# src-d/kmcuda

Measured on AMD Instinct MI355X. Metric: point-assignments/sec per Lloyd iter (8Mx256@1024), higher is better.
Workload: dtype f32

## Files before the change

kmcuda_amd/csrc/engine.cpp:

```cpp
#include "engine.hpp"

#include <math.h>
#include <stdio.h>
#include <stdlib.h>
#include <string.h>

#include <mutex>
#include <vector>

#include "../../include/kmcuda_amd.h"

namespace kmx {

int g_verbosity = 0;

namespace {
std::mutex g_stream_pool_mutex;
std::vector<std::vector<hipStream_t>> g_stream_pool;
}

hipStream_t pooled_stream_acquire(int device) {
  {
    std::lock_guard<std::mutex> lock(g_stream_pool_mutex);
    if ((size_t)device < g_stream_pool.size() && !g_stream_pool[device].empty()) {
// ... 43 lines not shown
  if (!pinned_) {
    if (hipHostMalloc(reinterpret_cast<void **>(&pinned_), kPinnedWords * sizeof(uint32_t), hipHostMallocCoherent) != hipSuccess) {
      pinned_ = nullptr;
      return nullptr;
    }
    memset(pinned_, 0, kPinnedWords * sizeof(uint32_t));
    void *dp = nullptr;
    if (hipHostGetDevicePointer(&dp, pinned_, 0) != hipSuccess || dp == nullptr) {
      (void)hipHostFree(pinned_);
      pinned_ = nullptr;
      pinned_dev_ = nullptr;
      return nullptr;
    }
    pinned_dev_ = static_cast<uint32_t *>(dp);
  }
  n = (n + 3u) & ~(size_t)3u;
  if (pinned_used_ + n > kPinnedWords) return nullptr;
  uint32_t *r = pinned_ + pinned_used_;
  if (dev_addr) *dev_addr = pinned_dev_ + pinned_used_;
  pinned_used_ += n;
  return r;
}

Engine::~Engine() {
  if (device_ >= 0) (void)hipSetDevice(device_);
  for (auto &s : spans_) { (void)hipEventDestroy(s.a); (void)hipEventDestroy(s.b); }
  for (void *p : owned_) (void)hipFree(p);
  if (pinned_) (void)hipHostFree(pinned_);
  if (side_stream_ && own_side_stream_) pooled_stream_release(device_, side_stream_);
  if (ev_fork_) (void)hipEventDestroy(ev_fork_);
  if (ev_join_) (void)hipEventDestroy(ev_join_);
  for (hipEvent_t e : ev_report_)
    if (e) (void)hipEventDestroy(e);
  if (ev_rows_) (void)hipEventDestroy(ev_rows_);
  if (own_stream_ && stream_) {
    if (blocking_stream_) (void)hipStreamDestroy(stream_);
    else pooled_stream_release(device_, stream_);
  }
}

int Engine::init(int device, uint32_t n_rows, uint32_t D, uint32_t K, int metric, int fp16x2, hipStream_t stream) {
  if (getenv("KMCUDA_AMD_DEBUG")) g_verbosity = atoi(getenv("KMCUDA_AMD_DEBUG"));
  if (const char *f = getenv("KMCUDA_AMD_FILTER")) filter_mode_ = strcmp(f, "f32") == 0 ? 1 : 0;
  if (const char *c = getenv("KMCUDA_AMD_ROW_CACHE")) row_cache_allowed_ = atoi(c) != 0;
  carry_pairs_ = true;
  if (const char *c = getenv("KMCUDA_AMD_CARRY_PAIRS")) carry_pairs_ = atoi(c) != 0;
  if (const char *c = getenv("KMCUDA_AMD_SETTLE")) settle_ = atoi(c) != 0;
  if (const char *c = getenv("KMCUDA_AMD_DUO")) { duo_on_ = atoi(c) != 0; duo_always_ = atoi(c) == 2; }
  if (const char *c = getenv("KMCUDA_AMD_COARSE_MFMA")) coarse_mfma_ = atoi(c) == 32 ? 32u : 16u;
  if (const char *c = getenv("KMCUDA_AMD_WIDE")) wide_ok_ = atoi(c) != 0;
  if (const char *c = getenv("KMCUDA_AMD_GEMM")) wide_ok_ = atoi(c) != 0;
  if (const char *u = getenv("KMCUDA_AMD_UPDATE"))
    ms_.force = strcmp(u, "radix") == 0 ? 1 : (strcmp(u, "sync") == 0 ? 2 : (strcmp(u, "bucket") == 0 ? 3 : 0));
  if (D == 0 || K < 1 || K >= 0x7FFFFFFFu) return kInvalidArguments;
  if (fp16x2) return kInvalidArguments;
  int ndev = 0;
  if (hipGetDeviceCount(&ndev) != hipSuccess || device < 0 || device >= ndev) return kNoSuchDevice;
  KMX_HIP(hipSetDevice(device), kNoSuchDevice);
  device_ = device;
  if (stream == (hipStream_t)(intptr_t)-1) {
    KMX_HIP(hipStreamCreateWithFlags(&stream_, hipStreamDefault), kRuntimeError);
    own_stream_ = true;
    blocking_stream_ = true;
  } else if (stream) {
    stream_ = stream;
  } else {
    stream_ = pooled_stream_acquire(device);
    if (!stream_) return kRuntimeError;
    own_stream_ = true;
  }
  N_ = n_rows; D_ = D; K_ = K; metric_ = metric; fp16x2_ = fp16x2;
  K_pad_ = (K + 31) / 32 * 32;
  Kt_ = (K + 63) / 64 * 64;
  DP_ = lloyd_dp_for(D);
  long wide_min_d = 257;
  if (const char *c = getenv("KMCUDA_AMD_WIDE_MIN_D")) {
    const long d = atol(c);
    if (d > 0) wide_min_d = d;
  }
  if (wide_ok_ && (long)D >= wide_min_d) DP_ = 0;
  eps_ = (float)(1.02 * ((double)D + 12.0) * ldexp(1.0, -24));
  tie_slack_ = metric == 0 ? 0.f : 1e-6f;

  wide_dp_ = (DP_ == 0 && wide_ok_) ? (D + 63) / 64 * 64 : 0;
  const uint32_t dp = DP_ ? DP_ : (wide_dp_ ? wide_dp_ : 8);
  int rc;
  if ((rc = alloc(&csqr_, K))) return rc;
  if ((rc = alloc(&bias_, K_pad_))) return rc;
  if ((rc = alloc(&bias2_, K_pad_))) return rc;
  if ((rc = alloc(&cfil_, (size_t)K_pad_ * dp))) return rc;
  if ((rc = alloc(&ct_, (size_t)D * Kt_))) return rc;
  if ((rc = alloc(&stats_base_, 16))) return rc;
  stats_ = stats_base_;
  if ((rc = alloc(&mu_, dp))) return rc;
  if ((rc = alloc(&finite_, Kt_))) return rc;
  if ((rc = alloc(&flagged_, n_rows))) return rc;
  if ((rc = alloc(&pairs_, 3 * (size_t)n_rows))) return rc;
  if ((rc = alloc(&counters_, 16))) return rc;
  if ((rc = alloc(&keys_tmp_, 2 * (size_t)n_rows))) return rc;
  if ((rc = alloc(&vals_tmp_, 2 * (size_t)n_rows))) return rc;
  if ((rc = alloc(&keys_sorted_, 2 * (size_t)n_rows))) return rc;
  if ((rc = alloc(&rows_sorted_, 2 * (size_t)n_rows))) return rc;
  if ((rc = alloc(&offsets2_, 2 * (size_t)K + 2))) return rc;
  if ((rc = alloc(&move_blocks_, (size_t)n_rows / 1024 + 4))) return rc;
  if ((rc = alloc(&bucket_work_, move_bucket_words(K)))) return rc;
  KMX_HIP(hipMemsetAsync(bucket_work_, 0, move_bucket_words(K) * sizeof(uint32_t), stream_), kRuntimeError);
// ... 1005 lines not shown
```

kmcuda_amd/csrc/kernels.hpp:

```cpp
#pragma once
#include <hip/hip_runtime.h>
#include <stdint.h>
#include "launch_dispatch.hpp"

namespace kmx {

struct LloydArgs {
  const float *samples;
  uint32_t N, D, K;
  uint32_t K_pad;
  uint32_t DP;
  uint32_t Kt;
  const float *cfil;
  const float *bias;
  const float *mu;
  const float *ct;
  const float *csqr;
  const uint32_t *stats;
  float eps;
  float tie_slack;
  uint32_t *assignments, *assignments_prev;
  uint32_t *flagged;
  uint32_t *pairs;
  uint32_t *counters;
// ... 45 lines not shown
                                       float *cfil, void *panelhi, uint32_t *stats, uint32_t *stats_next,
                                       uint32_t *zero_a, uint32_t *zero_b, uint32_t *zero_c,
                                       float *drift ,
                                       uint32_t *zero_d , hipStream_t st);
hipError_t launch_apply_prep_frozen(const double *delta, const double *dcount_d, float *centroids, uint32_t *ccounts,
                                    const StopCtl &stop, uint32_t K, uint32_t D, uint32_t K_pad, uint32_t DP,
                                    const float *mu, uint32_t *finite, float *bias, float *bias2, float *cfil,
                                    void *panelhi, uint32_t *stats, uint32_t *stats_next, uint32_t *zero_a,
                                    uint32_t *zero_b, uint32_t *zero_c, float *drift, uint32_t *zero_d, hipStream_t st);
hipError_t launch_lloyd_coarse_carry(const LloydArgs &a, const void *rows, bool half_rows, const void *xcache,
                                     const float *xmeta, const void *panelhi, uint32_t *undecided, float *und_thr,
                                     const CarryArgs &cy, uint32_t rows_hint, uint32_t *duo, hipStream_t st);
hipError_t launch_carry_skip(uint32_t N, uint32_t K, const uint32_t *assignments, uint32_t *assignments_prev,
                             const CarryArgs &cy, const float *xmeta, const float *drift, const uint32_t *stats,
                             float tie_slack, uint32_t *row_list, const uint32_t *finite, uint32_t *pairs,
                             uint32_t *counters, bool probe, hipStream_t st, uint32_t wide_dg = 0);
hipError_t launch_centroid_rows(int metric, const float *centroids, uint32_t K, uint32_t D, uint32_t Kt, float *csqr,
                                float *ct, hipStream_t st);
hipError_t launch_lloyd_coarse(const LloydArgs &a, const void *rows, bool half_rows, const void *xcache,
                               const float *xmeta, const void *panelhi, uint32_t *undecided, float *und_thr,
                               uint32_t *duo, hipStream_t st);
hipError_t launch_lloyd_duo(const LloydArgs &a, const uint32_t *duo, hipStream_t st, const CarryArgs *cy = nullptr);
hipError_t launch_lloyd_refine(const LloydArgs &a, const void *rows, bool half_rows, const void *panelhi,
                               const uint32_t *row_list, const float *thr_list, const uint32_t *n_list,
                               uint32_t rows_hint , hipStream_t st);
hipError_t launch_lloyd_refine_carry(const LloydArgs &a, const void *rows, bool half_rows, const void *panelhi,
                                     const uint32_t *row_list, const float *thr_list, const uint32_t *n_list,
                                     uint32_t rows_hint, const CarryArgs &cy, hipStream_t st);
hipError_t launch_row_cache(const void *rows, bool half_rows, uint32_t N, uint32_t D, uint32_t DP, const float *mu,
                            void *xcache, float *xmeta, hipStream_t st);

hipError_t launch_row_halves(const void *rows, bool half_rows, uint32_t N, uint32_t D, uint32_t DG, const float *mu,
                             void *xg, float *meta , hipStream_t st);
size_t wide_cont_words(uint32_t N);
hipError_t launch_lloyd_wide(const LloydArgs &a, const void *xg, const float *meta, uint32_t DG ,
                             const void *panelhi, uint32_t *undecided, float *und_thr, uint32_t *und_cont, hipStream_t st,
                             const CarryArgs *cy = nullptr);
hipError_t launch_wide_contenders(int metric, const LloydArgs &a, const float *centroids, uint32_t DG,
                                  const uint32_t *und_rows, const uint32_t *und_cont, hipStream_t st);

size_t sort_temp_bytes(size_t n, uint32_t max_key);
uint32_t move_bucket_stride(uint32_t K);
size_t move_bucket_words(uint32_t K);
uint32_t move_bucket_cap(uint32_t N, uint32_t K);
hipError_t launch_inverse_assignments(const uint32_t *assignments, uint32_t N, uint32_t K, uint32_t *keys_tmp,
                                      uint32_t *vals_tmp, uint32_t *keys_sorted, uint32_t *inv,
                                      uint32_t *offsets, void *temp, size_t temp_bytes, hipStream_t st);
struct MoveState {
  uint32_t *host = nullptr;
  uint32_t *host_dev = nullptr;
  uint32_t last_events = 0xFFFFFFFFu;
  int force = 0;
  uint32_t n_radix = 0, n_direct = 0;
};
struct MoveWeights {
  const float *weights;
  double *dweight;
  double *win;
};
hipError_t launch_move_deltas(const float *samples, uint32_t N, uint32_t D, uint32_t K, const uint32_t *prev,
                              const uint32_t *cur, uint32_t *keys_tmp, uint32_t *vals_tmp, uint32_t *keys_sorted,
                              uint32_t *rows_sorted, uint32_t *offsets2, void *temp, size_t temp_bytes,
                              uint32_t *bucket_rows, uint32_t cap, double *delta, int32_t *dcount ,
                              double *tail ,
                              const uint32_t *counters, uint32_t *blockoff, uint32_t *bucket_work, MoveState *ms,
                              hipStream_t st, const MoveWeights *mw = nullptr);
hipError_t launch_adjust_exact(int metric, const float *samples, uint32_t N, uint32_t D, uint32_t K,
                               const uint32_t *prev, const uint32_t *cur, uint32_t *keys_tmp, uint32_t *vals_tmp,
                               uint32_t *keys_sorted, uint32_t *rows_sorted, uint32_t *offsets2, void *temp,
                               size_t temp_bytes, float *work, float *centroids, uint32_t *ccounts, hipStream_t st);
hipError_t launch_apply_delta(int metric, const double *delta, const int32_t *dcount ,
                              const double *dcount_d , uint32_t K, uint32_t D,
                              float *centroids, uint32_t *ccounts, const StopCtl &stop, hipStream_t st,
                              const double *wtail = nullptr ,
                              double *cweights = nullptr );
size_t weights_check_doubles();
hipError_t launch_weights_check(const float *weights, uint32_t N, double *work, hipStream_t st);
hipError_t launch_sum_buffers(double *const *bufs_dev, uint32_t nbuf, size_t len, hipStream_t st);

hipError_t preload_update_code();
hipError_t preload_lloyd_f16_code();
hipError_t preload_lloyd_code();
hipError_t preload_lloyd_carry_code();
hipError_t preload_lloyd_duo_code();
hipError_t launch_gather_rows(const float *samples, const uint32_t *idx, uint32_t K, uint32_t D, float *out, hipStream_t st);
hipError_t launch_kmpp_step(int metric, const float *samples, uint32_t N, uint32_t D, const float *centroid,
                            uint32_t cc, float *dists, hipStream_t st);
struct KmppOutlierBuf {
  uint32_t *ecut = nullptr;
  void *outl = nullptr;
  uint32_t *outl_count = nullptr;
};
size_t kmpp_outlier_bytes();
size_t kmpp_totals_bytes();
hipError_t launch_kmpp_step2(int metric, const float *samples, uint32_t N, uint32_t D, const float *centroid,
                             uint32_t cc, float *dists, void *block_stats, double *bpre, void *totals,
                             const uint32_t *fail, const KmppOutlierBuf &out, hipStream_t st,
                             const float *weights = nullptr, float *terms = nullptr);
hipError_t launch_kmpp_weigh(const float *dists, const float *weights, uint32_t N, float *terms, const uint32_t *fail,
                             hipStream_t st);
constexpr int kKmppMaxShards = 16;
struct KmppShardPtrs {
  const float *dists;
  const double *bpre;
  void *totals;
  const float *samples;
// ... 295 lines not shown
```

kmcuda_amd/csrc/kmcuda_api.cpp:

```cpp
#include <dlfcn.h>
#include <math.h>
#include <stdio.h>
#include <stdlib.h>
#include <string.h>

#include <algorithm>
#include <chrono>
#include <cmath>
#include <condition_variable>
#include <functional>
#include <memory>
#include <mutex>
#include <thread>
#include <vector>

#include "../../include/kmcuda.h"
#include "../../include/kmcuda_amd.h"
#include "engine.hpp"
#include "knn_host.hpp"

using namespace kmx;

#define INFO(...) do { if (verbosity > 0) { printf(__VA_ARGS__); } } while (false)
#define DEBUG(...) do { if (verbosity > 1) { printf(__VA_ARGS__); } } while (false)
// ... 1499 lines not shown
  int ndev = 0;
  (void)hipGetDeviceCount(&ndev);
  return ndev < 32 && device > (1u << ndev);
}

void sync_callers_device(int32_t device_ptrs) {
  if (device_ptrs >= 0 && hipSetDevice(device_ptrs) == hipSuccess) (void)hipDeviceSynchronize();
}

int check_kmeans_args(const KmeansSwitches &sw, KMCUDAInitMethod init, float tolerance, float yinyang_t,
                      uint32_t samples_size, uint16_t features_size, uint32_t clusters_size, uint32_t device,
                      int32_t fp16x2, int32_t verbosity, const float *samples, const float *centroids,
                      const uint32_t *assignments, const float *sample_weights) {
  if (clusters_size < 2 || clusters_size == UINT32_MAX) return kmcudaInvalidArguments;
  if (features_size == 0) return kmcudaInvalidArguments;
  if (samples_size < clusters_size) return kmcudaInvalidArguments;
  if (device_mask_refused(device)) return kmcudaNoSuchDevice;
  if (samples == nullptr || centroids == nullptr || assignments == nullptr) return kmcudaInvalidArguments;
  if (tolerance < 0 || tolerance > 1) return kmcudaInvalidArguments;
  if (yinyang_t < 0 || yinyang_t > 0.5) return kmcudaInvalidArguments;
  if (!sample_weights) return kmcudaSuccess;
  if (init == kmcudaInitMethodAFKMC2 || sw.exact_update || (fp16x2 && sw.fp16_strict)) {
    INFO("sample weights are not supported with afkmc2, KMCUDA_AMD_EXACT_UPDATE=1 or KMCUDA_AMD_FP16_STRICT=1\n");
    return kmcudaInvalidArguments;
  }
  if (init == kmcudaInitMethodParallel) {
    INFO("sample weights are not supported with k-means||\n");
    return kmcudaInvalidArguments;
  }
  return kmcudaSuccess;
}

int seed_parallel_first(KMCUDAInitMethod *init, const void *init_params, KMCUDADistanceMetric metric,
                        uint32_t samples_size, uint16_t features_size, uint32_t clusters_size, uint32_t seed,
                        int first_device, int32_t device_ptrs, int32_t fp16x2, int32_t verbosity, const float *samples,
                        float *centroids) {
  if (*init != kmcudaInitMethodParallel) return kmcudaSuccess;
  const auto *sp = static_cast<const kmamd_seed_parallel_params *>(init_params);
  INFO("performing k-means||...\n");
  RETERR(kmamd_kmeans_seed_parallel(metric, samples_size, fp16x2 ? (uint16_t)(2u * features_size) : features_size,
                                    clusters_size, sp ? sp->rounds : 0u, sp ? sp->oversampling : 0.f, seed,
                                    device_ptrs >= 0 ? device_ptrs : first_device, device_ptrs, fp16x2, verbosity, samples,
                                    centroids, nullptr, nullptr, 0, nullptr, nullptr, nullptr));
  kmx::g_verbosity = verbosity;
  *init = kmcudaInitMethodImport;
  return kmcudaSuccess;
}

void publish_run_stats(Job &job, std::chrono::steady_clock::time_point t_loop) {
  job.stats.loop_seconds = std::chrono::duration<double>(std::chrono::steady_clock::now() - t_loop).count();
  job.collective_collect();
  if (job.sw.update_trace)
    for (auto &s : job.shards)
      fprintf(stderr, "[update] shard on device %d: %u radix, %u direct; loop %.4f s\n", s->dev, s->eng->ms_.n_radix, s->eng->ms_.n_direct,
              job.stats.loop_seconds);
  std::lock_guard<std::mutex> lock(g_last_run_mutex);
  g_last_run = job.stats;
}

}

extern "C" {

KMCUDAResult kmeans_cuda(KMCUDAInitMethod init, const void *init_params, float tolerance, float yinyang_t,
                         KMCUDADistanceMetric metric, uint32_t samples_size, uint16_t features_size,
                         uint32_t clusters_size, uint32_t seed, uint32_t device, int32_t device_ptrs, int32_t fp16x2,
                         int32_t verbosity, const float *samples, float *centroids, uint32_t *assignments,
                         float *average_distance) {
  return static_cast<KMCUDAResult>(kmamd_kmeans_weighted(init, init_params, tolerance, yinyang_t, metric, samples_size,
                                                         features_size, clusters_size, seed, device, device_ptrs, fp16x2,
                                                         verbosity, samples, centroids, assignments, average_distance,
                                                         nullptr));
}

int kmamd_kmeans_weighted(int init_, const void *init_params, float tolerance, float yinyang_t, int metric_,
                          uint32_t samples_size, uint16_t features_size, uint32_t clusters_size, uint32_t seed,
                          uint32_t device, int32_t device_ptrs, int32_t fp16x2, int32_t verbosity, const float *samples,
                          float *centroids, uint32_t *assignments, float *average_distance,
                          const float *sample_weights) {
  KMCUDAInitMethod init = static_cast<KMCUDAInitMethod>(init_);
  const KMCUDADistanceMetric metric = static_cast<KMCUDADistanceMetric>(metric_);
  kmx::g_verbosity = verbosity;
  DEBUG("arguments: %d %p %.3f %.2f %d %u %u %u %u %u %d %d %p %p %p %p\n", init, init_params, tolerance, yinyang_t,
        metric, samples_size, (unsigned)features_size, clusters_size, seed, device, fp16x2, verbosity,
        (const void *)samples, (void *)centroids, (void *)assignments, (void *)average_distance);
  const KmeansSwitches sw = kmeans_switches();
  RETERR(check_kmeans_args(sw, init, tolerance, yinyang_t, samples_size, features_size, clusters_size, device, fp16x2,
                           verbosity, samples, centroids, assignments, sample_weights));
  INFO("reassignments threshold: %u\n", uint32_t(tolerance * samples_size));
  const uint32_t yy_groups_size = yinyang_t * clusters_size;
  DEBUG("yinyang groups: %u\n", yy_groups_size);
  auto devs = setup_devices(device, verbosity);
  if (devs.empty()) return kmcudaNoSuchDevice;
  RETERR(seed_parallel_first(&init, init_params, metric, samples_size, features_size, clusters_size, seed, devs[0],
                             device_ptrs, fp16x2, verbosity, samples, centroids));
  sync_callers_device(device_ptrs);
  PreloadThreads preload;
  for (int d : devs) preload_code_objects(d, &preload, sw);
  PhaseClock clock(sw.timing);
  const auto t_begin = clock.t_lap;
  Job job;
  clock.wait = [&job] { (void)job.sync_all(); };
  job.fp16 = fp16x2 != 0;
  job.strict_h2 = job.fp16 && sw.fp16_strict;
  const uint32_t feats = fp16x2 ? 2u * features_size : features_size;
  RETERR(job.setup(sw, devs, sw.virtual_shards, samples_size, feats, clusters_size, metric, verbosity, samples,
                   device_ptrs, nullptr, sample_weights));
  clock.lap("set-up (engines, uploads)");
// ... 68 lines not shown
```

kmcuda_amd/csrc/list_sum.hpp:

```cpp
#pragma once
#include <hip/hip_runtime.h>
#include <stdint.h>

namespace kmx {

template <bool WEIGHTED>
__device__ __forceinline__ double list_sum(const float *__restrict__ samples, const float *__restrict__ weights,
                                           uint32_t D, const uint32_t *rows, uint32_t r0, uint32_t r1, uint32_t f) {
  double a[8] = {0, 0, 0, 0, 0, 0, 0, 0};
  uint32_t r = r0;
  for (; r + 8 <= r1; r += 8) {
    float x[8], w[8];
#pragma unroll
    for (int j = 0; j < 8; j++) {
      const uint32_t row = rows[r + j];
      x[j] = samples[(size_t)row * D + f];
      if constexpr (WEIGHTED) w[j] = weights[row];
    }
#pragma unroll
    for (int j = 0; j < 8; j++) {
      if constexpr (WEIGHTED) a[j] += (double)w[j] * (double)x[j];
      else a[j] += (double)x[j];
    }
  }
  for (uint32_t j = 0; r < r1; r++, j++) {
    const uint32_t row = rows[r];
    if constexpr (WEIGHTED) a[j] += (double)weights[row] * (double)samples[(size_t)row * D + f];
    else a[j] += (double)samples[(size_t)row * D + f];
  }
  return ((a[0] + a[1]) + (a[2] + a[3])) + ((a[4] + a[5]) + (a[6] + a[7]));
}

template <bool WEIGHTED>
__device__ __forceinline__ void list_sum4(const float *__restrict__ samples, const float *__restrict__ weights,
                                          uint32_t D, const uint32_t *rows, uint32_t r0, uint32_t r1, uint32_t f,
                                          double (&out)[4]) {
  double a[4][4];
#pragma unroll
  for (int j = 0; j < 4; j++)
#pragma unroll
    for (int e = 0; e < 4; e++) a[j][e] = 0.0;
  uint32_t r = r0;
  for (; r + 4 <= r1; r += 4) {
    float4 x[4];
    double w[4] = {1.0, 1.0, 1.0, 1.0};
#pragma unroll
    for (int j = 0; j < 4; j++) {
      const uint32_t row = rows[r + j];
      x[j] = *reinterpret_cast<const float4 *>(samples + (size_t)row * D + f);
      if constexpr (WEIGHTED) w[j] = (double)weights[row];
    }
#pragma unroll
    for (int j = 0; j < 4; j++) {
      if constexpr (WEIGHTED) {
        a[j][0] += w[j] * (double)x[j].x; a[j][1] += w[j] * (double)x[j].y;
        a[j][2] += w[j] * (double)x[j].z; a[j][3] += w[j] * (double)x[j].w;
      } else {
        a[j][0] += (double)x[j].x; a[j][1] += (double)x[j].y; a[j][2] += (double)x[j].z; a[j][3] += (double)x[j].w;
      }
    }
  }
  for (uint32_t j = 0; r < r1; r++, j++) {
    const uint32_t row = rows[r];
    float4 x = *reinterpret_cast<const float4 *>(samples + (size_t)row * D + f);
    double x0 = (double)x.x, x1 = (double)x.y, x2 = (double)x.z, x3 = (double)x.w;
    if constexpr (WEIGHTED) {
      const double w = (double)weights[row];
      x0 *= w; x1 *= w; x2 *= w; x3 *= w;
    }
    if (j == 0) { a[0][0] += x0; a[0][1] += x1; a[0][2] += x2; a[0][3] += x3; }
    else if (j == 1) { a[1][0] += x0; a[1][1] += x1; a[1][2] += x2; a[1][3] += x3; }
    else { a[2][0] += x0; a[2][1] += x1; a[2][2] += x2; a[2][3] += x3; }
  }
#pragma unroll
  for (int e = 0; e < 4; e++) out[e] = (a[0][e] + a[1][e]) + (a[2][e] + a[3][e]);
}

}
```

kmcuda_amd/csrc/update.hip:

```cpp
#include <stdio.h>
#include <stdlib.h>
#include <string.h>

#include <algorithm>

#include <rocprim/device/device_radix_sort.hpp>

#include "exact.hpp"
#include "kernels.hpp"
#include "list_sum.hpp"

namespace kmx {

static unsigned bits_for(uint64_t maxval) {
  unsigned b = 1;
  while (b < 32 && (1ull << b) <= maxval) b++;
  return b;
}

size_t sort_temp_bytes(size_t n, uint32_t max_key) {
  size_t bytes = 0;
  (void)rocprim::radix_sort_pairs(nullptr, bytes, (const uint32_t *)nullptr, (uint32_t *)nullptr,
                                  (const uint32_t *)nullptr, (uint32_t *)nullptr, n, 0u, bits_for(max_key),
                                  (hipStream_t)0);
// ... 222 lines not shown
    bool ein, eout;
    move_flags(prev, cur, s, N, K, p, a, ein, eout);
    const unsigned long long min = __ballot(ein), mout = __ballot(eout);
    const unsigned long long lower = (1ull << lane) - 1ull;
    const uint32_t rank = (uint32_t)__popcll(min & lower) + (uint32_t)__popcll(mout & lower);
    if (lane == 0) wcnt[wave] = (uint32_t)__popcll(min) + (uint32_t)__popcll(mout);
    __syncthreads();
    uint32_t wbase = 0, all = 0;
#pragma unroll
    for (uint32_t k = 0; k < 4; k++) {
      if (k < wave) wbase += wcnt[k];
      all += wcnt[k];
    }
    const size_t at = (size_t)off + wbase + rank;
    if (ein) { keys[at] = 2u * a; vals[at] = s; }
    if (eout) { keys[at + (ein ? 1 : 0)] = 2u * p + 1u; vals[at + (ein ? 1 : 0)] = s; }
    off += all;
    __syncthreads();
  }
}

constexpr uint32_t kSumThreads = 1024;
constexpr uint32_t kBucketCapMax = 4096;

uint32_t move_bucket_cap(uint32_t N, uint32_t K) {
  uint32_t cap = 32;
  while (cap < kBucketCapMax && (uint64_t)cap * 2 * K <= (uint64_t)N) cap <<= 1;
  return cap;
}

struct SumArgs {
  const float *samples;
  uint32_t N, D, K;
  const uint32_t *prev, *cur;
  uint32_t *cursors;
  uint32_t stride;
  const uint32_t *bucket_rows;
  uint32_t cap;
  uint32_t *overflow;
  const uint32_t *rows_sorted, *offsets2;
  double *delta;
  int32_t *dcount;
  double *tail;
  const uint32_t *counters;
  uint32_t *res;
  uint32_t *host;
};

struct SumWeightArgs {
  const float *weights;
  double *dweight;
  double *win;
};

template <bool DIRECT, bool VEC4, bool WEIGHTED>
__device__ __forceinline__ void cluster_sums_body(const SumArgs &a, const SumWeightArgs &wa) {
  extern __shared__ __attribute__((aligned(16))) unsigned char sums_lds[];
  double *part = reinterpret_cast<double *>(sums_lds);
  uint32_t (*srt)[kBucketCapMax] = reinterpret_cast<uint32_t (*)[kBucketCapMax]>(sums_lds + kSumThreads * 4 * sizeof(double));
  uint32_t *part_u = reinterpret_cast<uint32_t *>(part);
  __shared__ uint32_t wcnt[16];
  __shared__ uint32_t sh_base;
  const uint32_t c = blockIdx.x, tid = threadIdx.x, lane = tid & 63, wave = tid >> 6;
  const uint32_t D = a.D;
  const uint32_t *rows[2];
  uint32_t n[2];
  if (DIRECT) {
    n[0] = a.cursors[(size_t)(2 * c) * a.stride];
    n[1] = a.cursors[(size_t)(2 * c + 1) * a.stride];
    __syncthreads();
    if (tid < 2) a.cursors[(size_t)(2 * c + tid) * a.stride] = 0u;
#pragma unroll
    for (int sg = 0; sg < 2; sg++) {
      const uint32_t cnt = n[sg], key = 2 * c + sg;
      if (cnt <= kSumThreads && cnt <= a.cap) {
        uint32_t *v = srt[sg];
        const uint32_t mine = tid < cnt ? a.bucket_rows[(size_t)key * a.cap + tid] : 0xFFFFFFFFu;
        if (tid < cnt) part_u[tid] = mine;
        __syncthreads();
        if (tid < cnt) {
          uint32_t rank = 0;
          for (uint32_t j = 0; j < cnt; j++) rank += part_u[j] < mine ? 1u : 0u;
          v[rank] = mine;
        }
        __syncthreads();
        rows[sg] = v;
      } else if (cnt <= a.cap) {
        uint32_t m = 2;
        while (m < cnt) m <<= 1;
        uint32_t *v = srt[sg];
        for (uint32_t i = tid; i < m; i += kSumThreads) v[i] = i < cnt ? a.bucket_rows[(size_t)key * a.cap + i] : 0xFFFFFFFFu;
        __syncthreads();
        if (cnt > 1) {
          for (uint32_t k = 2; k <= m; k <<= 1) {
            for (uint32_t j = k >> 1; j > 0; j >>= 1) {
              for (uint32_t i = tid; i < m; i += kSumThreads) {
                const uint32_t l = i ^ j;
                if (l > i) {
                  const uint32_t x = v[i], y = v[l];
                  const bool up = (i & k) == 0;
                  if ((x > y) == up) { v[i] = y; v[l] = x; }
                }
              }
              __syncthreads();
            }
          }
// ... 85 lines not shown
        const uint32_t cnt = n[sg], chunk = (cnt + groups - 1) / groups;
        const uint32_t r0 = min(cnt, g * chunk), r1 = min(cnt, r0 + chunk);
        double mine[4] = {0.0, 0.0, 0.0, 0.0};
        if (fv && r1 > r0) list_sum4<WEIGHTED>(a.samples, wa.weights, D, rows[sg], r0, r1, f, mine);
#pragma unroll
        for (int e = 0; e < 4; e++) part[(size_t)tid * 4 + e] = mine[e];
        __syncthreads();
        if (g == 0) {
#pragma unroll
          for (int e = 0; e < 4; e++) {
            double t = part[(size_t)lf * 4 + e];
            for (uint32_t gg = 1; gg < groups; gg++) t += part[(size_t)(gg * fl + lf) * 4 + e];
            tot[sg][e] = t;
          }
        }
        __syncthreads();
      }
      if (g == 0 && fv) {
#pragma unroll
        for (int e = 0; e < 4; e++) a.delta[(size_t)c * D + f + e] = tot[0][e] - tot[1][e];
      }
    }
  } else {
  const uint32_t fl = D > 128 ? 256u : (D > 64 ? 128u : 64u), groups = kSumThreads / fl;
  const uint32_t g = tid / fl, lf = tid % fl;
  for (uint32_t f0 = 0; f0 < D; f0 += fl) {
    const uint32_t f = f0 + lf;
    const bool fv = f < D;
    double tot[2] = {0, 0};
#pragma unroll
    for (int sg = 0; sg < 2; sg++) {
      const uint32_t cnt = n[sg], chunk = (cnt + groups - 1) / groups;
      const uint32_t r0 = min(cnt, g * chunk), r1 = min(cnt, r0 + chunk);
      part[tid] = (fv && r1 > r0) ? list_sum<WEIGHTED>(a.samples, wa.weights, D, rows[sg], r0, r1, f) : 0.0;
      __syncthreads();
      if (g == 0) {
        double t = part[lf];
        for (uint32_t gg = 1; gg < groups; gg++) t += part[gg * fl + lf];
        tot[sg] = t;
      }
      __syncthreads();
    }
    if (g == 0 && fv) a.delta[(size_t)c * D + f] = tot[0] - tot[1];
  }
  }
  if (tid == 0) {
    const int32_t dc = (int32_t)n[0] - (int32_t)n[1];
    if (a.dcount) a.dcount[c] = dc;
    if (a.tail) a.tail[c] = (double)dc;
    if constexpr (WEIGHTED) {
      wa.dweight[c] = wsum[0] - wsum[1];
      wa.win[c] = wsum[0];
    }
    atomicAdd(&a.res[0], n[0] + n[1]);
    atomicMax(&a.res[1], max(n[0], n[1]));
    __threadfence();
    const uint32_t ticket = atomicAdd(&a.res[2], 1u);
    if (ticket == gridDim.x - 1) {
      if (a.counters[kStopFlag] == 0u) {
        volatile uint32_t *h = a.host;
        h[0] = atomicAdd(&a.res[0], 0u);
        h[1] = atomicAdd(&a.res[1], 0u);
        h[2] = a.counters[4];
        h[4] = a.counters[kDuoCount];
      }
      a.res[0] = 0u; a.res[1] = 0u; a.res[2] = 0u; a.res[3] = 0u;
    }
  }
  if (a.tail && c == 0 && tid < 4) a.tail[a.K + tid] = (double)a.counters[tid];
}

template <bool DIRECT, bool VEC4>
__global__ __launch_bounds__(kSumThreads) void cluster_sums_kernel(SumArgs a) {
  cluster_sums_body<DIRECT, VEC4, false>(a, SumWeightArgs{nullptr, nullptr, nullptr});
}
template <bool DIRECT, bool VEC4>
__global__ __launch_bounds__(kSumThreads) void cluster_sums_w_kernel(SumArgs a, SumWeightArgs wa) {
  cluster_sums_body<DIRECT, VEC4, true>(a, wa);
}

__global__ __launch_bounds__(256) void weight_changed_kernel(const double *__restrict__ win, uint32_t K,
                                                             double *__restrict__ out) {
  __shared__ double red[256];
  double t = 0.0;
  for (uint32_t c = threadIdx.x; c < K; c += 256) t += win[c];
  red[threadIdx.x] = t;
  __syncthreads();
  for (uint32_t s = 128; s > 0; s >>= 1) {
    if (threadIdx.x < s) red[threadIdx.x] += red[threadIdx.x + s];
    __syncthreads();
  }
  if (threadIdx.x == 0) out[0] = red[0];
}

constexpr uint32_t kWeightBlocks = 1024;
__global__ __launch_bounds__(256) void weights_check_kernel(const float *__restrict__ w, uint32_t N, uint32_t chunk,
                                                            double *__restrict__ part) {
  __shared__ double red[256], bad[256];
  const uint32_t lo = blockIdx.x * chunk, hi = min(N, lo + chunk);
  double t = 0.0, b = 0.0;
  for (uint32_t s = lo + threadIdx.x; s < hi; s += 256) {
    const float v = w[s];
    if (v > 0.f && v < INFINITY) t += (double)v; else b += 1.0;
  }
  red[threadIdx.x] = t; bad[threadIdx.x] = b;
  __syncthreads();
  for (uint32_t s = 128; s > 0; s >>= 1) {
    if (threadIdx.x < s) { red[threadIdx.x] += red[threadIdx.x + s]; bad[threadIdx.x] += bad[threadIdx.x + s]; }
    __syncthreads();
  }
  if (threadIdx.x == 0) { part[2 * blockIdx.x] = red[0]; part[2 * blockIdx.x + 1] = bad[0]; }
}
__global__ __launch_bounds__(256) void weights_total_kernel(const double *__restrict__ part, uint32_t nb,
                                                            double *__restrict__ out) {
  __shared__ double red[256], bad[256];
  double t = 0.0, b = 0.0;
  for (uint32_t i = threadIdx.x; i < nb; i += 256) { t += part[2 * i]; b += part[2 * i + 1]; }
  red[threadIdx.x] = t; bad[threadIdx.x] = b;
  __syncthreads();
  for (uint32_t s = 128; s > 0; s >>= 1) {
    if (threadIdx.x < s) { red[threadIdx.x] += red[threadIdx.x + s]; bad[threadIdx.x] += bad[threadIdx.x + s]; }
    __syncthreads();
  }
  if (threadIdx.x == 0) { out[0] = red[0]; out[1] = bad[0]; }
}
size_t weights_check_doubles() { return 2 * (size_t)kWeightBlocks + 2; }
hipError_t launch_weights_check(const float *weights, uint32_t N, double *work, hipStream_t st) {
  const uint32_t chunk = ((N + kWeightBlocks - 1) / kWeightBlocks + 255u) / 256u * 256u;
  const uint32_t nb = chunk ? (N + chunk - 1) / chunk : 0;
  if (nb) hipLaunchKernelGGL(weights_check_kernel, dim3(nb), dim3(256), 0, st, weights, N, chunk, work + 2);
  hipLaunchKernelGGL(weights_total_kernel, dim3(1), dim3(256), 0, st, work + 2, nb, work);
  return hipGetLastError();
}

uint32_t move_bucket_stride(uint32_t K) {
  uint32_t s = 32;
  while (s > 1 && 2ull * K * s > 262144ull) s >>= 1;
  return s;
}
size_t move_bucket_words(uint32_t K) { return 2 * (size_t)K * move_bucket_stride(K) + 4; }

__global__ __launch_bounds__(256) void move_scatter_kernel(const uint32_t *__restrict__ prev,
                                                           const uint32_t *__restrict__ cur, uint32_t N, uint32_t K,
                                                           uint32_t *__restrict__ cursors, uint32_t stride,
                                                           uint32_t *__restrict__ bucket_rows, uint32_t cap) {
  const uint32_t s = blockIdx.x * 256u + threadIdx.x;
  uint32_t p, a;
  bool ein, eout;
  move_flags(prev, cur, s, N, K, p, a, ein, eout);
  if (ein) {
    const uint32_t at = atomicAdd(&cursors[(size_t)(2u * a) * stride], 1u);
    if (at < cap) bucket_rows[(size_t)(2u * a) * cap + at] = s;
  }
  if (eout) {
    const uint32_t at = atomicAdd(&cursors[(size_t)(2u * p + 1u) * stride], 1u);
    if (at < cap) bucket_rows[(size_t)(2u * p + 1u) * cap + at] = s;
  }
}

hipError_t launch_move_deltas(const float *samples, uint32_t N, uint32_t D, uint32_t K, const uint32_t *prev,
                              const uint32_t *cur, uint32_t *keys_tmp, uint32_t *vals_tmp, uint32_t *keys_sorted,
                              uint32_t *rows_sorted, uint32_t *offsets2, void *temp, size_t temp_bytes,
                              uint32_t *bucket_rows, uint32_t cap, double *delta, int32_t *dcount, double *tail,
                              const uint32_t *counters, uint32_t *blockoff, uint32_t *bucket_work, MoveState *ms,
                              hipStream_t st, const MoveWeights *mw) {
  const uint32_t stride = move_bucket_stride(K);
  SumArgs a;
  a.samples = samples; a.N = N; a.D = D; a.K = K; a.prev = prev; a.cur = cur;
  a.cursors = bucket_work; a.stride = stride; a.bucket_rows = bucket_rows; a.cap = cap;
  a.overflow = rows_sorted; a.rows_sorted = rows_sorted; a.offsets2 = offsets2;
  a.delta = delta; a.dcount = dcount; a.tail = tail; a.counters = counters;
  a.res = bucket_work + 2 * (size_t)K * stride; a.host = ms->host_dev;
  hipError_t e = hipSuccess;
  const bool vec4 = (D & 3u) == 0 && (((uintptr_t)samples) & 15u) == 0;
  const size_t sums_lds = kSumThreads * 4 * sizeof(double) + 2 * kBucketCapMax * sizeof(uint32_t);
  auto launch_sums = [&](bool direct) {
    if (mw) {
      const SumWeightArgs wa{mw->weights, mw->dweight, mw->win};
      const void *fn = direct ? (vec4 ? (const void *)cluster_sums_w_kernel<true, true> : (const void *)cluster_sums_w_kernel<true, false>)
                              : (vec4 ? (const void *)cluster_sums_w_kernel<false, true> : (const void *)cluster_sums_w_kernel<false, false>);
      if (hipFuncSetAttribute(fn, hipFuncAttributeMaxDynamicSharedMemorySize, (int)sums_lds) != hipSuccess) return;
      if (direct) {
        if (vec4) hipLaunchKernelGGL((cluster_sums_w_kernel<true, true>), dim3(K), dim3(kSumThreads), sums_lds, st, a, wa);
        else hipLaunchKernelGGL((cluster_sums_w_kernel<true, false>), dim3(K), dim3(kSumThreads), sums_lds, st, a, wa);
      } else {
        if (vec4) hipLaunchKernelGGL((cluster_sums_w_kernel<false, true>), dim3(K), dim3(kSumThreads), sums_lds, st, a, wa);
        else hipLaunchKernelGGL((cluster_sums_w_kernel<false, false>), dim3(K), dim3(kSumThreads), sums_lds, st, a, wa);
      }
      hipLaunchKernelGGL(weight_changed_kernel, dim3(1), dim3(256), 0, st, mw->win, K, mw->dweight + K);
      return;
    }
    const void *fn = direct ? (vec4 ? (const void *)cluster_sums_kernel<true, true> : (const void *)cluster_sums_kernel<true, false>)
                            : (vec4 ? (const void *)cluster_sums_kernel<false, true> : (const void *)cluster_sums_kernel<false, false>);
    if (hipFuncSetAttribute(fn, hipFuncAttributeMaxDynamicSharedMemorySize, (int)sums_lds) != hipSuccess) return;
    if (direct) {
      if (vec4) hipLaunchKernelGGL((cluster_sums_kernel<true, true>), dim3(K), dim3(kSumThreads), sums_lds, st, a);
      else hipLaunchKernelGGL((cluster_sums_kernel<true, false>), dim3(K), dim3(kSumThreads), sums_lds, st, a);
    } else {
      if (vec4) hipLaunchKernelGGL((cluster_sums_kernel<false, true>), dim3(K), dim3(kSumThreads), sums_lds, st, a);
      else hipLaunchKernelGGL((cluster_sums_kernel<false, false>), dim3(K), dim3(kSumThreads), sums_lds, st, a);
    }
  };
  const bool force_radix = ms->force == 1, force_sync = ms->force == 2, force_direct = ms->force == 3;
  const uint32_t est_max = std::max((uint32_t)ms->host[1] , ms->last_events / K);
  const bool radix = N != 0 && !force_direct &&
                     (force_radix || ms->last_events > N / 2 || est_max > cap - cap / 4);
  if (N == 0) {
    e = hipMemsetAsync(offsets2, 0, (2 * (size_t)K + 1) * sizeof(uint32_t), st);
    if (e != hipSuccess) return e;
    launch_sums(false);
  } else if (radix) {
    ms->n_radix++;
    const uint32_t nb = (N + kMoveRows - 1) / kMoveRows;
    hipLaunchKernelGGL(move_count_kernel, dim3(nb), dim3(256), 0, st, prev, cur, N, K, blockoff);
    hipLaunchKernelGGL(move_scan_kernel, dim3(1), dim3(1024), 0, st, blockoff, nb, blockoff + nb + 1);
    hipLaunchKernelGGL(move_write_kernel, dim3(nb), dim3(256), 0, st, prev, cur, N, K, blockoff, keys_tmp, vals_tmp);
    e = hipGetLastError();
    if (e != hipSuccess) return e;
    e = hipMemcpyAsync(ms->host + 3, blockoff + nb + 1, sizeof(uint32_t), hipMemcpyDeviceToHost, st);
    if (e == hipSuccess) e = hipStreamSynchronize(st);
    if (e != hipSuccess) return e;
    const uint32_t m = ms->host[3];
    if (m) {
      e = rocprim::radix_sort_pairs(temp, temp_bytes, (const uint32_t *)keys_tmp, keys_sorted,
                                    (const uint32_t *)vals_tmp, rows_sorted, (size_t)m, 0u, bits_for(2ull * K), st);
      if (e != hipSuccess) return e;
    }
    hipLaunchKernelGGL(offsets_kernel, dim3((2 * K + 1 + 255) / 256), dim3(256), 0, st, keys_sorted, m, 2 * K, offsets2);
    ms->last_events = m;
    ms->host[0] = m;
    launch_sums(false);
  } else {
    ms->n_direct++;
    hipLaunchKernelGGL(move_scatter_kernel, dim3((N + 255) / 256), dim3(256), 0, st, prev, cur, N, K, bucket_work,
                       stride, bucket_rows, cap);
    launch_sums(true);
    e = hipGetLastError();
    if (e != hipSuccess) return e;
    if (force_sync) {
      e = hipStreamSynchronize(st);
      if (e != hipSuccess) return e;
    }
    ms->last_events = ms->host[0];
  }
  return hipGetLastError();
}

template <int METRIC, bool WEIGHTED>
__device__ __forceinline__ void apply_delta_body(const double *__restrict__ delta, const int32_t *__restrict__ dcount,
                                                 const double *__restrict__ dcount_d, uint32_t D,
                                                 float *__restrict__ centroids, uint32_t *__restrict__ ccounts,
                                                 const StopCtl &ctl, const double *__restrict__ wtail,
                                                 double *__restrict__ cweights) {
  const uint32_t c = blockIdx.x;
  if (ctl.counters) {
    bool stop = ctl.counters[kStopFlag] != 0u;
    if constexpr (WEIGHTED) {
      if (ctl.threshold >= 0.f && dcount_d) stop = stop || (float)wtail[gridDim.x] <= ctl.threshold;
    } else {
      if (ctl.threshold >= 0.f && dcount_d) stop = stop || (float)(uint32_t)dcount_d[gridDim.x] <= ctl.threshold;
    }
    if (c == 0 && threadIdx.x == 0) {
      if (stop) ctl.counters[kStopFlag] = 1u;
      else if (ctl.threshold >= 0.f) ctl.counters[0] = 0u;
      if (ctl.host_tail) {
        volatile uint32_t *ht = ctl.host_tail;
        for (uint32_t i = 0; i < 4; i++) ht[i] = dcount_d ? (uint32_t)dcount_d[gridDim.x + i] : 0u;
        ht[4] = stop ? 1u : 0u;
        __threadfence_system();
        ht[5] = ctl.seq;
      }
    }
    if (stop) return;
  }
  const double *d = delta + (size_t)c * D;
  float *cen = centroids + (size_t)c * D;
  const uint32_t cnt_old = ccounts[c];
  const uint32_t cnt_new = cnt_old + (uint32_t)(dcount_d ? (int32_t)dcount_d[c] : dcount[c]);
  double w, cn;
  if constexpr (WEIGHTED) {
    w = cnt_old ? cweights[c] : 0.0;
    cn = w + wtail[c];
  } else {
    w = (double)cnt_old;
    cn = (double)cnt_new;
  }
  if (cnt_new == 0) {
    for (uint32_t f = threadIdx.x; f < D; f += blockDim.x) cen[f] = __builtin_nanf("");
  } else if (METRIC == 0) {
// ... 167 lines not shown
```

Before: 2.199 billion.

## Add two-wave per-cluster sums kernel and vectorize move scatter

Adds a 128-thread cluster_sums_wave_kernel in which one wave sums a cluster's incoming rows and the other its outgoing rows, using readlane-broadcast row ids, multiple double accumulators and in-LDS rank or bitonic sorting of bucket rows. It is used when the estimated per-cluster move list is small, and it merges the completion counters into a single 64-bit atomic. The move scatter kernel now handles four rows per thread with uint4 loads, which cuts the launched thread count. The aim is lower sums-stage cost in late Lloyd iterations where few points move, at the price of a large new code path with sort and overflow handling.

Result: no change. 2.215 billion (median of 6 runs) (+0.7%).

```diff
diff --git a/kmcuda_amd/csrc/engine.cpp b/kmcuda_amd/csrc/engine.cpp
--- a/kmcuda_amd/csrc/engine.cpp
+++ b/kmcuda_amd/csrc/engine.cpp
@@ -119,6 +119,8 @@
   if (const char *c = getenv("KMCUDA_AMD_GEMM")) wide_ok_ = atoi(c) != 0;
   if (const char *u = getenv("KMCUDA_AMD_UPDATE"))
     ms_.force = strcmp(u, "radix") == 0 ? 1 : (strcmp(u, "sync") == 0 ? 2 : (strcmp(u, "bucket") == 0 ? 3 : 0));
+  if (const char *u = getenv("KMCUDA_AMD_SUMS"))
+    ms_.sums = strcmp(u, "block") == 0 ? 1 : (strcmp(u, "wave-always") == 0 ? 2 : 0);
   if (D == 0 || K < 1 || K >= 0x7FFFFFFFu) return kInvalidArguments;
   if (fp16x2) return kInvalidArguments;
   int ndev = 0;
diff --git a/kmcuda_amd/csrc/kernels.hpp b/kmcuda_amd/csrc/kernels.hpp
--- a/kmcuda_amd/csrc/kernels.hpp
+++ b/kmcuda_amd/csrc/kernels.hpp
@@ -121,6 +121,8 @@
   uint32_t last_events = 0xFFFFFFFFu;
   int force = 0;
   uint32_t n_radix = 0, n_direct = 0;
+  int sums = 0;
+  uint32_t n_wave = 0;
 };
 struct MoveWeights {
   const float *weights;
diff --git a/kmcuda_amd/csrc/kmcuda_api.cpp b/kmcuda_amd/csrc/kmcuda_api.cpp
--- a/kmcuda_amd/csrc/kmcuda_api.cpp
+++ b/kmcuda_amd/csrc/kmcuda_api.cpp
@@ -1575,8 +1575,8 @@
   job.collective_collect();
   if (job.sw.update_trace)
     for (auto &s : job.shards)
-      fprintf(stderr, "[update] shard on device %d: %u radix, %u direct; loop %.4f s\n", s->dev, s->eng->ms_.n_radix, s->eng->ms_.n_direct,
-              job.stats.loop_seconds);
+      fprintf(stderr, "[update] shard on device %d: %u radix, %u direct, %u summed per wave; loop %.4f s\n", s->dev,
+              s->eng->ms_.n_radix, s->eng->ms_.n_direct, s->eng->ms_.n_wave, job.stats.loop_seconds);
   std::lock_guard<std::mutex> lock(g_last_run_mutex);
   g_last_run = job.stats;
 }
diff --git a/kmcuda_amd/csrc/list_sum.hpp b/kmcuda_amd/csrc/list_sum.hpp
--- a/kmcuda_amd/csrc/list_sum.hpp
+++ b/kmcuda_amd/csrc/list_sum.hpp
@@ -76,4 +76,90 @@
   for (int e = 0; e < 4; e++) out[e] = (a[0][e] + a[1][e]) + (a[2][e] + a[3][e]);
 }
 
+template <int V>
+__device__ __forceinline__ void row_load(const float *__restrict__ p, float (&x)[V]) {
+  if constexpr (V == 4) {
+    const float4 v = *reinterpret_cast<const float4 *>(p);
+    x[0] = v.x; x[1] = v.y; x[2] = v.z; x[3] = v.w;
+  } else {
+    x[0] = *p;
+  }
 }
+
+template <int V, int A, int NB, bool LROWS>
+__device__ __forceinline__ void wave_list_sum(const float *__restrict__ samples, uint32_t D, const uint32_t *rows,
+                                              uint32_t n, uint32_t groups, uint32_t f, double (&tot)[V]) {
+  static_assert(64 % NB == 0 && (A == 4 || A == 8), "window and accumulators");
+  typedef const __attribute__((address_space(3))) uint32_t *lds_rows_t;
+#pragma unroll
+  for (int e = 0; e < V; e++) tot[e] = 0.0;
+  if (n == 0) return;
+  const uint32_t lane = threadIdx.x & 63;
+  const uint32_t chunk = (n + groups - 1) / groups;
+  double acc[A][V], t[V];
+#pragma unroll
+  for (int q = 0; q < A; q++)
+#pragma unroll
+    for (int e = 0; e < V; e++) acc[q][e] = 0.0;
+#pragma unroll
+  for (int e = 0; e < V; e++) t[e] = 0.0;
+  auto ids = [&](uint32_t at) -> uint32_t {
+    const uint32_t i = min(at + lane, n - 1);
+    if constexpr (LROWS) return ((lds_rows_t)rows)[i];
+    else return rows[i];
+  };
+  uint32_t bb = 0;
+  uint32_t idc = ids(0), idn = ids(64);
+  float x[NB][V];
+#pragma unroll
+  for (int j = 0; j < NB; j++) {
+    const uint32_t row = (uint32_t)__builtin_amdgcn_readlane((int)idc, (int)min((uint32_t)j, n - 1));
+    row_load<V>(samples + (size_t)row * D + f, x[j]);
+  }
+  uint32_t pos = 0, glen = min(chunk, n), folded = 0;
+  for (uint32_t i0 = 0; i0 < n; i0 += NB) {
+    if (i0 == bb + 64) { bb += 64; idc = idn; idn = ids(bb + 64); }
+#pragma unroll
+    for (int j = 0; j < NB; j++) {
+      const uint32_t i = i0 + j;
+      double xd[V];
+#pragma unroll
+      for (int e = 0; e < V; e++) xd[e] = (double)x[j][e];
+      {
+        const uint32_t k = min(i + NB, n - 1) - bb;
+        const uint32_t r0 = (uint32_t)__builtin_amdgcn_readlane((int)idc, (int)(k & 63u));
+        const uint32_t r1 = (uint32_t)__builtin_amdgcn_readlane((int)idn, (int)(k & 63u));
+        const uint32_t row = k < 64u ? r0 : r1;
+        row_load<V>(samples + (size_t)row * D + f, x[j]);
+      }
+      if (i < n) {
+        const uint32_t sel = pos & (uint32_t)(A - 1);
+#pragma unroll
+        for (int q = 0; q < A; q++) {
+          if (sel == (uint32_t)q) {
+#pragma unroll
+            for (int e = 0; e < V; e++) acc[q][e] += xd[e];
+          }
+        }
+        if (++pos == glen) {
+#pragma unroll
+          for (int e = 0; e < V; e++) {
+            double s;
+            if constexpr (A == 4) s = (acc[0][e] + acc[1][e]) + (acc[2][e] + acc[3][e]);
+            else s = ((acc[0][e] + acc[1][e]) + (acc[2][e] + acc[3][e])) + ((acc[4][e] + acc[5][e]) + (acc[6][e] + acc[7][e]));
+            t[e] = folded ? t[e] + s : s;
+#pragma unroll
+            for (int q = 0; q < A; q++) acc[q][e] = 0.0;
+          }
+          folded++;
+          pos = 0;
+          glen = min(chunk, n - i - 1);
+        }
+      }
+    }
+  }
+#pragma unroll
+  for (int e = 0; e < V; e++) tot[e] = folded < groups ? t[e] + 0.0 : t[e];
+}
+
+}
diff --git a/kmcuda_amd/csrc/update.hip b/kmcuda_amd/csrc/update.hip
--- a/kmcuda_amd/csrc/update.hip
+++ b/kmcuda_amd/csrc/update.hip
@@ -298,6 +298,23 @@
   double *dweight;
   double *win;
 };
+
+__device__ __forceinline__ void sums_report(const SumArgs &a, uint32_t n_in, uint32_t n_out) {
+  atomicAdd(&a.res[0], n_in + n_out);
+  atomicMax(&a.res[1], max(n_in, n_out));
+  __threadfence();
+  const uint32_t ticket = atomicAdd(&a.res[2], 1u);
+  if (ticket == gridDim.x - 1) {
+    if (a.counters[kStopFlag] == 0u) {
+      volatile uint32_t *h = a.host;
+      h[0] = atomicAdd(&a.res[0], 0u);
+      h[1] = atomicAdd(&a.res[1], 0u);
+      h[2] = a.counters[4];
+      h[4] = a.counters[kDuoCount];
+    }
+    a.res[0] = 0u; a.res[1] = 0u; a.res[2] = 0u; a.res[3] = 0u;
+  }
+}
 
 template <bool DIRECT, bool VEC4, bool WEIGHTED>
 __device__ __forceinline__ void cluster_sums_body(const SumArgs &a, const SumWeightArgs &wa) {
@@ -489,20 +506,7 @@
       wa.dweight[c] = wsum[0] - wsum[1];
       wa.win[c] = wsum[0];
     }
-    atomicAdd(&a.res[0], n[0] + n[1]);
-    atomicMax(&a.res[1], max(n[0], n[1]));
-    __threadfence();
-    const uint32_t ticket = atomicAdd(&a.res[2], 1u);
-    if (ticket == gridDim.x - 1) {
-      if (a.counters[kStopFlag] == 0u) {
-        volatile uint32_t *h = a.host;
-        h[0] = atomicAdd(&a.res[0], 0u);
-        h[1] = atomicAdd(&a.res[1], 0u);
-        h[2] = a.counters[4];
-        h[4] = a.counters[kDuoCount];
-      }
-      a.res[0] = 0u; a.res[1] = 0u; a.res[2] = 0u; a.res[3] = 0u;
-    }
+    sums_report(a, n[0], n[1]);
   }
   if (a.tail && c == 0 && tid < 4) a.tail[a.K + tid] = (double)a.counters[tid];
 }
@@ -514,6 +518,175 @@
 template <bool DIRECT, bool VEC4>
 __global__ __launch_bounds__(kSumThreads) void cluster_sums_w_kernel(SumArgs a, SumWeightArgs wa) {
   cluster_sums_body<DIRECT, VEC4, true>(a, wa);
+}
+
+constexpr uint32_t kWaveThreads = 128;
+constexpr uint32_t kWaveRank = 256;
+constexpr uint32_t kWaveListMax = 1024;
+
+template <int V, int A, int NB, bool LROWS>
+__device__ __forceinline__ void wave_sums_slabs(const SumArgs &a, uint32_t c, uint32_t wave, uint32_t lane,
+                                                const uint32_t *rows, uint32_t n, uint32_t groups, double *xch) {
+  for (uint32_t f0 = 0; f0 < a.D; f0 += 64u * V) {
+    const uint32_t f = f0 + lane * V;
+    const bool fv = f < a.D;
+    double tot[V];
+    wave_list_sum<V, A, NB, LROWS>(a.samples, a.D, rows, n, groups, fv ? f : 0u, tot);
+    if (wave == 1) {
+#pragma unroll
+      for (int e = 0; e < V; e++) xch[lane * V + e] = tot[e];
+    }
+    __syncthreads();
+    if (wave == 0 && fv) {
+#pragma unroll
+      for (int e = 0; e < V; e++) a.delta[(size_t)c * a.D + f + e] = tot[e] - xch[lane * V + e];
+    }
+    __syncthreads();
+  }
+}
+template <int V, int A, int NB>
+__device__ __forceinline__ void wave_sums_run(const SumArgs &a, uint32_t c, uint32_t wave, uint32_t lane,
+                                              const uint32_t *rows_g, const uint32_t *rows_l, uint32_t n,
+                                              uint32_t groups, double *xch) {
+  if (rows_g) wave_sums_slabs<V, A, NB, false>(a, c, wave, lane, rows_g, n, groups, xch);
+  else wave_sums_slabs<V, A, NB, true>(a, c, wave, lane, rows_l, n, groups, xch);
+}
+
+__device__ __forceinline__ void wave_report(const SumArgs &a, uint32_t n_in, uint32_t n_out) {
+  uint32_t z = atomicMax(&a.res[2], max(n_in, n_out));
+  asm volatile("v_and_b32 %0, 0, %0" : "+v"(z));
+  const unsigned long long mine = ((unsigned long long)(n_in + n_out) << 32) + 1ull + z;
+  const unsigned long long old = atomicAdd(reinterpret_cast<unsigned long long *>(a.res), mine);
+  if ((uint32_t)old == gridDim.x - 1) {
+    if (a.counters[kStopFlag] == 0u) {
+      volatile uint32_t *h = a.host;
+      h[0] = (uint32_t)(old >> 32) + n_in + n_out;
+      h[1] = atomicAdd(&a.res[2], 0u);
+      h[2] = a.counters[4];
+      h[4] = a.counters[kDuoCount];
+    }
+    a.res[0] = 0u; a.res[1] = 0u; a.res[2] = 0u; a.res[3] = 0u;
+  }
+}
+
+template <bool DIRECT, bool VEC4>
+__global__ __launch_bounds__(kWaveThreads) void cluster_sums_wave_kernel(SumArgs a) {
+  __shared__ __attribute__((aligned(16))) uint32_t srt[2][kBucketCapMax];
+  __shared__ double xch[64 * 4];
+  const uint32_t c = blockIdx.x, tid = threadIdx.x, lane = tid & 63;
+  const uint32_t wave = (uint32_t)__builtin_amdgcn_readfirstlane((int)(tid >> 6));
+  uint32_t n[2];
+  const uint32_t *rows_g = nullptr;
+  if (DIRECT) {
+    n[0] = (uint32_t)__builtin_amdgcn_readfirstlane((int)a.cursors[(size_t)(2 * c) * a.stride]);
+    n[1] = (uint32_t)__builtin_amdgcn_readfirstlane((int)a.cursors[(size_t)(2 * c + 1) * a.stride]);
+    __syncthreads();
+    if (tid < 2) a.cursors[(size_t)(2 * c + tid) * a.stride] = 0u;
+    const uint32_t cnt = n[wave], key = 2 * c + wave;
+    uint32_t *v = srt[wave];
+    const int mode = cnt > a.cap ? 2 : (cnt > kWaveRank ? 1 : 0);
+    uint32_t m = 0;
+    if (mode == 0) m = (cnt + 3u) & ~3u;
+    if (mode == 1) { m = 2; while (m < cnt) m <<= 1; }
+    for (uint32_t i = lane; i < m; i += 64) v[i] = i < cnt ? a.bucket_rows[(size_t)key * a.cap + i] : 0xFFFFFFFFu;
+    __syncthreads();
+    uint32_t mine[4], rank[4] = {0, 0, 0, 0};
+    if (mode == 0) {
+#pragma unroll
+      for (int k = 0; k < 4; k++) mine[k] = lane + 64u * k < cnt ? v[lane + 64u * k] : 0u;
+      for (uint32_t j = 0; j < m; j += 4) {
+        const uint4 o = *reinterpret_cast<const uint4 *>(v + j);
+#pragma unroll
+        for (int k = 0; k < 4; k++)
+          rank[k] += (o.x < mine[k] ? 1u : 0u) + (o.y < mine[k] ? 1u : 0u) + (o.z < mine[k] ? 1u : 0u) + (o.w < mine[k] ? 1u : 0u);
+      }
+    }
+    __syncthreads();
+    if (mode == 0) {
+#pragma unroll
+      for (int k = 0; k < 4; k++)
+        if (lane + 64u * k < cnt) v[rank[k]] = mine[k];
+    }
+    const uint32_t n0 = n[0] > kWaveRank && n[0] <= a.cap ? n[0] : 0u, n1 = n[1] > kWaveRank && n[1] <= a.cap ? n[1] : 0u;
+    const uint32_t longest = max(n0, n1);
+    if (longest) {
+      uint32_t mm = 2;
+      while (mm < longest) mm <<= 1;
+      for (uint32_t k = 2; k <= mm; k <<= 1) {
+        for (uint32_t j = k >> 1; j > 0; j >>= 1) {
+          if (mode == 1 && k <= m) {
+            for (uint32_t i = lane; i < m; i += 64) {
+              const uint32_t l = i ^ j;
+              if (l > i) {
+                const uint32_t x = v[i], y = v[l];
+                const bool up = (i & k) == 0;
+                if ((x > y) == up) { v[i] = y; v[l] = x; }
+              }
+            }
+          }
+          __syncthreads();
+        }
+      }
+    }
+    if (mode == 2) {
+      uint32_t base_w = 0;
+      if (lane == 0) base_w = atomicAdd(&a.res[3], cnt);
+      base_w = (uint32_t)__builtin_amdgcn_readfirstlane((int)base_w);
+      uint32_t *dst = a.overflow + base_w;
+      uint32_t done = 0;
+      for (uint64_t base = 0; base < a.N; base += 256) {
+        uint32_t hit[4], cntme = 0;
+#pragma unroll
+        for (uint32_t q = 0; q < 4; q++) {
+          const uint64_t s64 = base + lane * 4 + q;
+          const uint32_t s = s64 < a.N ? (uint32_t)s64 : a.N;
+          uint32_t p, cu;
+          bool ein, eout;
+          move_flags(a.prev, a.cur, s, a.N, a.K, p, cu, ein, eout);
+          const bool hitme = wave == 0 ? (ein && cu == c) : (eout && p == c);
+          hit[q] = hitme ? s : 0xFFFFFFFFu;
+          cntme += hitme ? 1u : 0u;
+        }
+        uint32_t inc = cntme;
+#pragma unroll
+        for (int o = 1; o < 64; o <<= 1) {
+          const uint32_t t = __shfl_up(inc, o);
+          if ((int)lane >= o) inc += t;
+        }
+        uint32_t at = done + inc - cntme;
+#pragma unroll
+        for (uint32_t q = 0; q < 4; q++)
+          if (hit[q] != 0xFFFFFFFFu) dst[at++] = hit[q];
+        done += (uint32_t)__builtin_amdgcn_readlane((int)inc, 63);
+      }
+      __threadfence();
+      rows_g = dst;
+    }
+    __syncthreads();
+  } else {
+    const uint32_t o0 = a.offsets2[2 * c], o1 = a.offsets2[2 * c + 1], o2 = a.offsets2[2 * c + 2];
+    n[0] = (uint32_t)__builtin_amdgcn_readfirstlane((int)(o1 - o0));
+    n[1] = (uint32_t)__builtin_amdgcn_readfirstlane((int)(o2 - o1));
+    rows_g = a.rows_sorted + (wave == 0 ? o0 : o1);
+  }
+
+  const uint32_t D = a.D, cnt = n[wave];
+  if (VEC4 && max(n[0], n[1]) >= 128u) {
+    uint32_t fl = 16;
+    while (fl < 256u && fl * 4u < D) fl <<= 1;
+    wave_sums_run<4, 4, 16>(a, c, wave, lane, rows_g, srt[wave], cnt, kSumThreads / fl, xch);
+  } else {
+    const uint32_t fl = D > 128 ? 256u : (D > 64 ? 128u : 64u);
+    if (VEC4) wave_sums_run<4, 8, 8>(a, c, wave, lane, rows_g, srt[wave], cnt, kSumThreads / fl, xch);
+    else wave_sums_run<1, 8, 8>(a, c, wave, lane, rows_g, srt[wave], cnt, kSumThreads / fl, xch);
+  }
+  if (tid == 0) {
+    const int32_t dc = (int32_t)n[0] - (int32_t)n[1];
+    if (a.dcount) a.dcount[c] = dc;
+    if (a.tail) a.tail[c] = (double)dc;
+    wave_report(a, n[0], n[1]);
+  }
+  if (a.tail && c == 0 && tid < 4) a.tail[a.K + tid] = (double)a.counters[tid];
 }
 
 __global__ __launch_bounds__(256) void weight_changed_kernel(const double *__restrict__ win, uint32_t K,
@@ -580,19 +753,36 @@
 __global__ __launch_bounds__(256) void move_scatter_kernel(const uint32_t *__restrict__ prev,
                                                            const uint32_t *__restrict__ cur, uint32_t N, uint32_t K,
                                                            uint32_t *__restrict__ cursors, uint32_t stride,
-                                                           uint32_t *__restrict__ bucket_rows, uint32_t cap) {
-  const uint32_t s = blockIdx.x * 256u + threadIdx.x;
-  uint32_t p, a;
-  bool ein, eout;
-  move_flags(prev, cur, s, N, K, p, a, ein, eout);
-  if (ein) {
-    const uint32_t at = atomicAdd(&cursors[(size_t)(2u * a) * stride], 1u);
-    if (at < cap) bucket_rows[(size_t)(2u * a) * cap + at] = s;
-  }
-  if (eout) {
-    const uint32_t at = atomicAdd(&cursors[(size_t)(2u * p + 1u) * stride], 1u);
-    if (at < cap) bucket_rows[(size_t)(2u * p + 1u) * cap + at] = s;
-  }
+                                                           uint32_t *__restrict__ bucket_rows, uint32_t cap, int vec16) {
+  const uint64_t s0 = ((uint64_t)blockIdx.x * 256u + threadIdx.x) * 4u;
+  if (s0 >= N) return;
+  uint32_t p[4], a[4];
+  if (vec16 && s0 + 4 <= N) {
+    const uint4 pv = *reinterpret_cast<const uint4 *>(prev + s0), av = *reinterpret_cast<const uint4 *>(cur + s0);
+    p[0] = pv.x; p[1] = pv.y; p[2] = pv.z; p[3] = pv.w;
+    a[0] = av.x; a[1] = av.y; a[2] = av.z; a[3] = av.w;
+  } else {
+#pragma unroll
+    for (uint32_t q = 0; q < 4; q++) {
+      p[q] = a[q] = 0;
+      if (s0 + q < N) { p[q] = prev[s0 + q]; a[q] = cur[s0 + q]; }
+    }
+  }
+  uint32_t key[8], at[8];
+#pragma unroll
+  for (uint32_t q = 0; q < 4; q++) {
+    const bool moved = p[q] != a[q];
+    key[2 * q] = moved && a[q] < K ? 2u * a[q] : 0xFFFFFFFFu;
+    key[2 * q + 1] = moved && p[q] < K ? 2u * p[q] + 1u : 0xFFFFFFFFu;
+  }
+#pragma unroll
+  for (uint32_t e = 0; e < 8; e++) {
+    at[e] = cap;
+    if (key[e] != 0xFFFFFFFFu) at[e] = atomicAdd(&cursors[(size_t)key[e] * stride], 1u);
+  }
+#pragma unroll
+  for (uint32_t e = 0; e < 8; e++)
+    if (at[e] < cap) bucket_rows[(size_t)key[e] * cap + at[e]] = (uint32_t)s0 + (e >> 1);
 }
 
 hipError_t launch_move_deltas(const float *samples, uint32_t N, uint32_t D, uint32_t K, const uint32_t *prev,
@@ -611,7 +801,18 @@
   hipError_t e = hipSuccess;
   const bool vec4 = (D & 3u) == 0 && (((uintptr_t)samples) & 15u) == 0;
   const size_t sums_lds = kSumThreads * 4 * sizeof(double) + 2 * kBucketCapMax * sizeof(uint32_t);
-  auto launch_sums = [&](bool direct) {
+  auto launch_sums = [&](bool direct, uint32_t est) {
+    if (!mw && ms->sums != 1 && (ms->sums == 2 || est <= kWaveListMax)) {
+      if (direct) {
+        if (vec4) hipLaunchKernelGGL((cluster_sums_wave_kernel<true, true>), dim3(K), dim3(kWaveThreads), 0, st, a);
+        else hipLaunchKernelGGL((cluster_sums_wave_kernel<true, false>), dim3(K), dim3(kWaveThreads), 0, st, a);
+      } else {
+        if (vec4) hipLaunchKernelGGL((cluster_sums_wave_kernel<false, true>), dim3(K), dim3(kWaveThreads), 0, st, a);
+        else hipLaunchKernelGGL((cluster_sums_wave_kernel<false, false>), dim3(K), dim3(kWaveThreads), 0, st, a);
+      }
+      ms->n_wave++;
+      return;
+    }
     if (mw) {
       const SumWeightArgs wa{mw->weights, mw->dweight, mw->win};
       const void *fn = direct ? (vec4 ? (const void *)cluster_sums_w_kernel<true, true> : (const void *)cluster_sums_w_kernel<true, false>)
@@ -645,7 +846,7 @@
   if (N == 0) {
     e = hipMemsetAsync(offsets2, 0, (2 * (size_t)K + 1) * sizeof(uint32_t), st);
     if (e != hipSuccess) return e;
-    launch_sums(false);
+    launch_sums(false, 0u);
   } else if (radix) {
     ms->n_radix++;
     const uint32_t nb = (N + kMoveRows - 1) / kMoveRows;
@@ -666,12 +867,13 @@
     hipLaunchKernelGGL(offsets_kernel, dim3((2 * K + 1 + 255) / 256), dim3(256), 0, st, keys_sorted, m, 2 * K, offsets2);
     ms->last_events = m;
     ms->host[0] = m;
-    launch_sums(false);
+    launch_sums(false, std::max((uint32_t)ms->host[1], 2 * (m / K)));
   } else {
     ms->n_direct++;
-    hipLaunchKernelGGL(move_scatter_kernel, dim3((N + 255) / 256), dim3(256), 0, st, prev, cur, N, K, bucket_work,
-                       stride, bucket_rows, cap);
-    launch_sums(true);
+    const int vec16 = ((((uintptr_t)prev) | ((uintptr_t)cur)) & 15u) == 0 ? 1 : 0;
+    hipLaunchKernelGGL(move_scatter_kernel, dim3((N + 1023) / 1024), dim3(256), 0, st, prev, cur, N, K, bucket_work,
+                       stride, bucket_rows, cap, vec16);
+    launch_sums(true, est_max);
     e = hipGetLastError();
     if (e != hipSuccess) return e;
     if (force_sync) {
```
